# shivangchopra11/MedMoE

Measured on AMD Instinct MI355X. Metric: image-text pairs/sec at global batch 1024, higher is better.
Workload: dtype bf16; 1 GPU; cfg2: ViT-B/16 + 12-layer text tower (frozen), 8 experts top-2, 224x224x3 + 77 tokens, fwd+bwd+clip+Adam; global_batch=1024, per_gpu_batch=1024, parallelism=dp1

## Files before the change

### medmoe_amd/csrc/gemm_scores.hip

```cpp
#include "gemm_nt.h"
#include "options.h"

struct ScoresArgs {
  const bf16_t* ctx; const bf16_t* words; const int* cap_lens; const int* cap_list;
  bf16_t* a1; float* lse;
  int M, HW, HWP, Bc, T, D, n_cap;
  long long col_base, ldp, bstride;
  int skip_epi; float inv_hw;
};

template <int CTRL>
__device__ __forceinline__ float sc_dpp(float v) {
  return __builtin_bit_cast(float, __builtin_amdgcn_update_dpp(0, __builtin_bit_cast(int, v), CTRL, 0xf, 0xf, true));
}
__device__ __forceinline__ float sc_row16_sum(float v) {
  v += sc_dpp<0xB1>(v); v += sc_dpp<0x4E>(v); v += sc_dpp<0x141>(v); v += sc_dpp<0x140>(v);
  return v;
}
__device__ __forceinline__ float sc_row16_max(float v) {
  v = fmaxf(v, sc_dpp<0xB1>(v)); v = fmaxf(v, sc_dpp<0x4E>(v)); v = fmaxf(v, sc_dpp<0x141>(v)); v = fmaxf(v, sc_dpp<0x140>(v));
  return v;
}

#define SC_DPP4(OP, CTRL)                                                                                            \
  "v_" OP "_f32_dpp %0, %0, %0 " CTRL " row_mask:0xf bank_mask:0xf\n\tv_" OP "_f32_dpp %1, %1, %1 " CTRL " row_mask:0xf bank_mask:0xf\n\t" \
  "v_" OP "_f32_dpp %2, %2, %2 " CTRL " row_mask:0xf bank_mask:0xf\n\tv_" OP "_f32_dpp %3, %3, %3 " CTRL " row_mask:0xf bank_mask:0xf\n\t"
__device__ __forceinline__ void sc_row16_max4(float& a, float& b, float& c, float& d) {
  asm volatile("s_nop 1\n\t" SC_DPP4("max", "quad_perm:[1,0,3,2]") SC_DPP4("max", "quad_perm:[2,3,0,1]") SC_DPP4("max", "row_half_mirror")
               SC_DPP4("max", "row_mirror") : "+v"(a), "+v"(b), "+v"(c), "+v"(d));
}
__device__ __forceinline__ void sc_row16_sum4(float& a, float& b, float& c, float& d) {
  asm volatile("s_nop 1\n\t" SC_DPP4("add", "quad_perm:[1,0,3,2]") SC_DPP4("add", "quad_perm:[2,3,0,1]") SC_DPP4("add", "row_half_mirror")
               SC_DPP4("add", "row_mirror") : "+v"(a), "+v"(b), "+v"(c), "+v"(d));
}

template <int NTT, bool TR = false>
__global__ __launch_bounds__(512, 2) void scores512_kernel(ScoresArgs p) {
  constexpr int TP = NTT * 16;
  constexpr int WNN = (NTT == 5) ? 2 : 4;
  constexpr int WMM = 8 / WNN;
  constexpr int TMW = 16 / WMM;
  constexpr int CW = (NTT == 1) ? 4 : (NTT == 2) ? 2 : 1;
  constexpr int TNW = CW * NTT;
  constexpr int BNS = WNN * TNW * 16;
  constexpr int CAPB = WNN * CW;
  constexpr int NPIECE = (256 + BNS) / 16;
  __shared__ __attribute__((aligned(16))) char smem[NRING * SUB3];
  const int tid = threadIdx.x, lane = tid & 63, wid = tid >> 6;
  const int wm = wid % WMM, wn = wid / WMM;
  const int fr = lane & 15, g = lane >> 4;
  const int G = gridDim.x;
  const int my = xcd_remap(blockIdx.x, G);
  const int tiles_m = (p.M + 255) / 256, tiles_n = (p.n_cap + CAPB - 1) / CAPB;
  const int total = tiles_m * tiles_n;
  const int nu = p.D / 32;
  struct Tile { int m0, c0; };
  auto decode = [&](int id) -> Tile { Tile t; t.m0 = (id / tiles_n) * 256; t.c0 = (id % tiles_n) * CAPB; return t; };

  unsigned src[4];
  bool have[4];
  auto setup = [&](const Tile& t) {
#pragma unroll
    for (int i = 0; i < 4; ++i) {
      const int piece = i * 8 + wid;
      have[i] = piece < NPIECE;
      const int line = piece * 8 + (lane >> 3);
      const int lc = (lane & 7) ^ (line & 7);
      const int row = 2 * line + (lc >> 2);
      if (i < 2) src[i] = (unsigned)min(t.m0 + row, p.M - 1) * (unsigned)(p.D * 2) + (lc & 3) * 16;
      else {
        const int n = min(row - 256, BNS - 1);
        const int cj = min(t.c0 + n / TP, p.n_cap - 1), tw = min(n % TP, p.T - 1);
        src[i] = (unsigned)(p.cap_list[cj] * p.T + tw) * (unsigned)(p.D * 2) + (lc & 3) * 16;
      }
    }
  };
  auto stage = [&](int buf, int k0) {
    char* sb = smem + buf * SUB3 + wid * 1024;
#pragma unroll
    for (int i = 0; i < 4; ++i)
      if (have[i])
        __builtin_amdgcn_global_load_lds(GLB_PTR((const char*)(i < 2 ? p.ctx : p.words) + k0 * 2 + src[i]), LDS_PTR(sb + i * 8192), 16, 0, 0);
  };
  f32x4_t acc[TMW][TNW];
  auto zero_acc = [&]() __attribute__((always_inline)) {
#pragma unroll
    for (int i = 0; i < TMW; ++i)
#pragma unroll
      for (int j = 0; j < TNW; ++j) acc[i][j] = (f32x4_t){0.f, 0.f, 0.f, 0.f};
  };
  const int lane_off = (fr >> 1) * 128 + (((((fr & 1) << 2) | g) ^ ((fr >> 1) & 7)) << 4);
  const int offA_nat = (wm * TMW * 16) * 64 + lane_off;
  const int sig = ((((fr >> 2) & 1) << 1 | (fr >> 3)) << 2) | (fr & 3);
  const int pg = ((g & 1) << 1) | (g >> 1);
  const int sig_off = (sig >> 1) * 128 + (((((sig & 1) << 2) | g) ^ ((sig >> 1) & 7)) << 4);
  const int offA = TR ? (wm * TMW * 16) * 64 + sig_off : offA_nat;
  const int offB = (256 + wn * TNW * 16) * 64 + (TR ? lane_off : sig_off);
  bf16x8_t af[TMW], bf[TNW];
  auto read_frags = [&](int buf) __attribute__((always_inline)) {
    const char* sA = smem + buf * SUB3 + offA;
    const char* sB = smem + buf * SUB3 + offB;
#pragma unroll
    for (int t = 0; t < TMW; ++t) af[t] = *(const bf16x8_t*)(sA + t * 1024);
#pragma unroll
    for (int t = 0; t < TNW; ++t) bf[t] = *(const bf16x8_t*)(sB + t * 1024);
  };
  auto compute = [&]() __attribute__((always_inline)) {
#pragma unroll
    for (int tm = 0; tm < TMW; ++tm)
#pragma unroll
      for (int tn = 0; tn < TNW; ++tn)
        acc[tm][tn] = TR ? __builtin_amdgcn_mfma_f32_16x16x32_bf16(af[tm], bf[tn], acc[tm][tn], 0, 0, 0)
                         : __builtin_amdgcn_mfma_f32_16x16x32_bf16(bf[tn], af[tm], acc[tm][tn], 0, 0, 0);
  };
  auto div_hw = [&](int m, int& q, int& r) __attribute__((always_inline)) {
    q = (int)(((float)m + 0.5f) * p.inv_hw);
    r = m - q * p.HW;
    if (r < 0) { --q; r += p.HW; }
    if (r >= p.HW) { ++q; r -= p.HW; }
  };
  auto epilogue_t = [&](const Tile& t) __attribute__((always_inline)) {
#pragma unroll
    for (int c = 0; c < CW; ++c) {
      const int cj = t.c0 + wn * CW + c;
      const bool cap_ok = cj < p.n_cap && p.skip_epi != 2;
      const int cap_i = p.cap_list[min(cj, p.n_cap - 1)];
      const int cap = max(1, min(min(p.cap_lens[cap_i], p.T), TP));
      if ((NTT - 1) * 16 + fr >= cap) {
#pragma unroll
        for (int tm = 0; tm < TMW; ++tm)
#pragma unroll
          for (int r = 0; r < 4; ++r) acc[tm][c * NTT + NTT - 1][r] = -INFINITY;
      }
      if (NTT > 1 && cap <= (NTT - 1) * 16) {
#pragma unroll
        for (int tn = 0; tn < NTT - 1; ++tn)
          if (tn * 16 + fr >= cap) {
#pragma unroll
            for (int tm = 0; tm < TMW; ++tm)
#pragma unroll
              for (int r = 0; r < 4; ++r) acc[tm][c * NTT + tn][r] = -INFINITY;
          }
      }
#pragma unroll
      for (int J = 0; J < TMW / 4; ++J) {
        uint4 vv[2][NTT];
#pragma unroll
        for (int jq = 0; jq < 2; ++jq) {
          const int jp = 2 * J + jq;
          uint2 o[2][NTT];
#pragma unroll
          for (int q = 0; q < 2; ++q) {
            const int tm = 2 * jp + q;
            constexpr float L2E = 1.44269504088896f;
            float mx[4], sm[4], lse2[4];
  #pragma unroll
            for (int r = 0; r < 4; ++r) {
              mx[r] = acc[tm][c * NTT][r];
  #pragma unroll
              for (int tn = 1; tn < NTT; ++tn) mx[r] = fmaxf(mx[r], acc[tm][c * NTT + tn][r]);
            }
            sc_row16_max4(mx[0], mx[1], mx[2], mx[3]);
  #pragma unroll
            for (int r = 0; r < 4; ++r) {
              mx[r] *= L2E;
              sm[r] = 0.f;
  #pragma unroll
              for (int tn = 0; tn < NTT; ++tn) sm[r] += __builtin_amdgcn_exp2f(__builtin_fmaf(acc[tm][c * NTT + tn][r], L2E, -mx[r]));
            }
            sc_row16_sum4(sm[0], sm[1], sm[2], sm[3]);
            float lse4[4];
  #pragma unroll
            for (int r = 0; r < 4; ++r) { lse2[r] = mx[r] + __builtin_amdgcn_logf(sm[r]); lse4[r] = lse2[r] * 0.6931471805599453f; }
            typedef _Float16 h2_t __attribute__((ext_vector_type(2)));
            const h2_t lo2 = __builtin_bit_cast(h2_t, LOGP_MIN_BITS2);
  #pragma unroll
            for (int tn = 0; tn < NTT; ++tn) {
              float e[4];
  #pragma unroll
              for (int r = 0; r < 4; ++r) e[r] = __builtin_fmaf(acc[tm][c * NTT + tn][r], L2E, -lse2[r]);
              o[q][tn].x = __builtin_bit_cast(uint32_t, __builtin_elementwise_max(__builtin_bit_cast(h2_t, pack2h(e[0], e[1])), lo2));
              o[q][tn].y = __builtin_bit_cast(uint32_t, __builtin_elementwise_max(__builtin_bit_cast(h2_t, pack2h(e[2], e[3])), lo2));
            }
            const int m4 = t.m0 + wm * TMW * 16 + tm * 16 + 4 * pg;
            if (fr == 0 && m4 < p.M && cap_ok) {
              int mb, hw;
              div_hw(m4, mb, hw);
              *(float4*)(p.lse + ((long long)mb * p.Bc + cap_i) * p.HWP + hw) = make_float4(lse4[0], lse4[1], lse4[2], lse4[3]);
            }
          }
  
#pragma unroll
          for (int tn = 0; tn < NTT; ++tn) {
            auto r0 = __builtin_amdgcn_permlane32_swap(o[0][tn].x, o[1][tn].x, false, false);
            auto r1 = __builtin_amdgcn_permlane32_swap(o[0][tn].y, o[1][tn].y, false, false);
            vv[jq][tn] = make_uint4(r0[0], r1[0], r0[1], r1[1]);
          }
        }
        const int m8 = t.m0 + wm * TMW * 16 + (4 * J + (g >> 1)) * 16 + (g & 1) * 8 + 32 * (fr >> 3);
        int mb, hw;
        div_hw(min(m8, p.M - 4), mb, hw);
        const bool ok = m8 < p.M && cap_ok;
        const bool whole = hw + 8 <= p.HW;
        const bool ok2 = m8 + 4 < p.M;
        bf16_t* dst0 = p.a1 + (p.col_base + (long long)cj * TP + (fr & 7)) * p.ldp + (long long)mb * p.bstride + hw;
        bf16_t* dst2 = p.a1 + (p.col_base + (long long)cj * TP + (fr & 7)) * p.ldp + (long long)(mb + 1) * p.bstride;
#pragma unroll
        for (int tn = 0; tn < NTT; ++tn) {
#pragma unroll
          for (int i = 0; i < 2; ++i) {
            const uint4 a = vv[0][tn], b = vv[1][tn];
            uint4 y;
            if (i == 0) {
              y.x = __builtin_amdgcn_update_dpp(a.x, b.x, 0x128, 0xf, 0xC, false); y.y = __builtin_amdgcn_update_dpp(a.y, b.y, 0x128, 0xf, 0xC, false);
              y.z = __builtin_amdgcn_update_dpp(a.z, b.z, 0x128, 0xf, 0xC, false); y.w = __builtin_amdgcn_update_dpp(a.w, b.w, 0x128, 0xf, 0xC, false);
            } else {
              y.x = __builtin_amdgcn_update_dpp(b.x, a.x, 0x128, 0xf, 0x3, false); y.y = __builtin_amdgcn_update_dpp(b.y, a.y, 0x128, 0xf, 0x3, false);
              y.z = __builtin_amdgcn_update_dpp(b.z, a.z, 0x128, 0xf, 0x3, false); y.w = __builtin_amdgcn_update_dpp(b.w, a.w, 0x128, 0xf, 0x3, false);
            }
            const long long ro = (long long)(tn * 16 + 8 * i) * p.ldp;
            if (ok && whole) *(uint4*)(dst0 + ro) = y;
            else if (ok) {
              *(uint2*)(dst0 + ro) = make_uint2(y.x, y.y);
              if (ok2) *(uint2*)(dst2 + ro) = make_uint2(y.z, y.w);
            }
          }
        }
      }
    }
  };
  auto epilogue = [&](const Tile& t) __attribute__((always_inline)) -> int {
    int n_st = 0;
#pragma unroll
    for (int c = 0; c < CW; ++c) {
      const int cj = t.c0 + wn * CW + c;
      const bool cap_ok = cj < p.n_cap;
      const int cap_i = p.cap_list[min(cj, p.n_cap - 1)];
      const int cap = min(min(p.cap_lens[cap_i], p.T), TP);
#pragma unroll
      for (int tm = 0; tm < TMW; ++tm) {
        float mx = -INFINITY;
#pragma unroll
        for (int tn = 0; tn < NTT; ++tn)
#pragma unroll
          for (int r = 0; r < 4; ++r)
            if (tn * 16 + pg * 4 + r < cap) mx = fmaxf(mx, acc[tm][c * NTT + tn][r]);
        mx = fmaxf(mx, __shfl_xor(mx, 16, 64));
        mx = fmaxf(mx, __shfl_xor(mx, 32, 64));
        float sm = 0.f;
#pragma unroll
        for (int tn = 0; tn < NTT; ++tn)
#pragma unroll
          for (int r = 0; r < 4; ++r)
            sm += (tn * 16 + pg * 4 + r < cap) ? __expf(acc[tm][c * NTT + tn][r] - mx) : 0.f;
        sm += __shfl_xor(sm, 16, 64);
        sm += __shfl_xor(sm, 32, 64);
        const float lse = mx + __logf(sm);
        const int m = t.m0 + wm * TMW * 16 + tm * 16 + fr;
        const bool ok = m < p.M && cap_ok;
        const int mb = min(m, p.M - 1) / p.HW, hw = min(m, p.M - 1) - mb * p.HW;
        if (ok && g == 0) p.lse[((long long)mb * p.Bc + cap_i) * p.HWP + hw] = lse;
        bf16_t* dst = p.a1 + ((long long)mb * p.HWP + hw) * p.ldp + p.col_base + (long long)cj * TP;
        float e[NTT][4];
#pragma unroll
        for (int tn = 0; tn < NTT; ++tn)
#pragma unroll
          for (int r = 0; r < 4; ++r)
            e[tn][r] = (tn * 16 + pg * 4 + r < cap) ? fmaxf(acc[tm][c * NTT + tn][r] - lse, LOGP_MIN) : LOGP_MIN;
        uint2 o[NTT];
#pragma unroll
        for (int tn = 0; tn < NTT; ++tn) {
          o[tn].x = pack2h(e[tn][0], e[tn][1]);
          o[tn].y = pack2h(e[tn][2], e[tn][3]);
        }
#pragma unroll
        for (int j = 0; j < NTT / 2; ++j) {
          auto r0 = __builtin_amdgcn_permlane32_swap(o[2 * j].x, o[2 * j + 1].x, false, false);
          auto r1 = __builtin_amdgcn_permlane32_swap(o[2 * j].y, o[2 * j + 1].y, false, false);
          if (ok) *(uint4*)(dst + (2 * j + (g >> 1)) * 16 + (g & 1) * 8) = make_uint4(r0[0], r1[0], r0[1], r1[1]);
        }
        if ((NTT & 1) && ok) *(uint2*)(dst + (NTT - 1) * 16 + pg * 4) = o[NTT - 1];
        n_st += NTT;
      }
    }
    return n_st + TMW * CW;
  };

  if (my >= total) return;
  const int my_tiles = (total - my + G - 1) / G;
  Tile ct = decode(my);
  setup(ct);
  int lid = my, lk = 0, wb = 0, rb = 0;
  bool lmore = true;
  int drain = 0;
  auto issue = [&]() __attribute__((always_inline)) {
    if (lmore) {
      stage(wb, lk * 32);
      wb = (wb + 1) & 3;
      if (++lk == nu) {
        lk = 0; lid += G;
        if (lid < total) { const Tile lt = decode(lid); setup(lt); } else lmore = false;
      }
    }
  };
  const int my_pieces = (have[0] ? 1 : 0) + (have[1] ? 1 : 0) + (have[2] ? 1 : 0) + (have[3] ? 1 : 0);
  auto wait_third_newest = [&]() __attribute__((always_inline)) {
    if (drain > 0 || !lmore) { asm volatile("s_waitcnt vmcnt(0)" ::: "memory"); if (drain > 0) --drain; }
    else if (my_pieces == 4) asm volatile("s_waitcnt vmcnt(8)" ::: "memory");
    else if (my_pieces == 3) asm volatile("s_waitcnt vmcnt(6)" ::: "memory");
    else asm volatile("s_waitcnt vmcnt(4)" ::: "memory");
  };
  const int grp = __builtin_amdgcn_readfirstlane(wid >> 2);
  zero_acc();
  issue(); issue(); issue();
  asm volatile("s_waitcnt vmcnt(0)" ::: "memory");
  __builtin_amdgcn_s_barrier();
  asm volatile("" ::: "memory");
  auto seg_barrier = [&]() {
    __builtin_amdgcn_sched_barrier(0);
    __builtin_amdgcn_s_barrier();
    __builtin_amdgcn_sched_barrier(0);
    asm volatile("" ::: "memory");
  };
  auto load_seg = [&]() __attribute__((always_inline)) {
    read_frags(rb);
    rb = (rb + 1) & 3;
    issue();
    if (grp == 1) wait_third_newest();
    seg_barrier();
  };
  auto body = [&](bool last) __attribute__((always_inline)) {
    compute();
    if (grp == 0) { wait_third_newest(); seg_barrier(); }
    if (last) {
      if (p.skip_epi != 1) { if constexpr (TR) epilogue_t(ct); else epilogue(ct); }
      zero_acc();
      drain = 3;
    }
    if (grp == 1) seg_barrier();
    load_seg();
  };
  if (grp == 1) seg_barrier();
  load_seg();
  for (int ti = 0; ti < my_tiles; ++ti) {
    for (int k = 1; k < nu; ++k) body(false);
    body(true);
    if (ti + 1 < my_tiles) ct = decode(my + (ti + 1) * G);
  }
  if (grp == 0) seg_barrier();
}

int g_use_scores512 = 1, g_scores_skip_epi = 0;

static ScoresArgs sc_args(const void* ctx, const void* words, const int* cap_lens, const int* cap_list, void* out, float* lse, long long M,
                          int HW, int Bc, int T, int D, int n_cap, long long col_base, long long ldp, long long bstride) {
  ScoresArgs p;
  p.ctx = (const bf16_t*)ctx; p.words = (const bf16_t*)words; p.cap_lens = cap_lens; p.cap_list = cap_list;
  p.a1 = (bf16_t*)out; p.lse = lse;
  p.M = (int)M; p.HW = HW; p.HWP = ((HW + 15) / 16) * 16; p.Bc = Bc; p.T = T; p.D = D; p.n_cap = n_cap;
  p.col_base = col_base; p.ldp = ldp; p.bstride = bstride; p.skip_epi = g_scores_skip_epi; p.inv_hw = 1.0f / (float)HW;
  return p;
}

template <bool TR>
static void sc_launch(const ScoresArgs& p, int ntt, hipStream_t stream) {
  const int tiles_m = (p.M + 255) / 256;
#define SC(N_, CAPB_) { const int grid = min(tiles_m * ((p.n_cap + CAPB_ - 1) / CAPB_), 256); \
                        hipLaunchKernelGGL((scores512_kernel<N_, TR>), dim3(grid), dim3(512), 0, stream, p); }
  switch (ntt) { case 1: SC(1, 16) break; case 2: SC(2, 8) break; case 3: SC(3, 4) break; case 4: SC(4, 4) break; default: SC(5, 2) break; }
#undef SC
}

extern "C" int medmoe_local_scores_t(const void* ctx, const void* words, const int* cap_lens, void* lpT, float* lse, int B, int Bc,
                                     int HW, int T, int D, const int* cap_list, int n_cap, int ntt, long long row_base, long long ld,
                                     long long bstride, hipStream_t stream) {
  if (!ctx || !words || !cap_lens || !lpT || !lse || !cap_list) return MM_ERR_ARG;
  if (B <= 0 || Bc <= 0 || HW < 4 || (HW % 4) || T <= 0 || n_cap <= 0 || n_cap > Bc || ntt < 1 || ntt > 5 || row_base < 0) return MM_ERR_SHAPE;
  const long long M = (long long)B * HW;
  const int HWP = ((HW + 15) / 16) * 16;
  if ((D % 32) || D < 128 || M * D * 2 >= (1ll << 32) || (long long)Bc * T * D * 2 >= (1ll << 32) || (ld % 4) || (bstride % 4) || ld < HWP || bstride < HWP) return MM_ERR_SHAPE;
  sc_launch<true>(sc_args(ctx, words, cap_lens, cap_list, lpT, lse, M, HW, Bc, T, D, n_cap, row_base, ld, bstride), ntt, stream);
  return mm_check_launch();
}

bool mm_launch_scores512(const void* ctx, const void* words, const int* cap_lens, void* a1, float* lse, int B, int Bc, int HW, int T,
                         int D, const int* cap_list, int n_cap, int ntt, long long col_base, long long ldp, hipStream_t stream) {
  const long long M = (long long)B * HW;
  if (!g_use_scores512 || (D % 32) || D < 128 || M < 1024 || M * D * 2 >= (1ll << 32) || (long long)Bc * T * D * 2 >= (1ll << 32)) return false;
  sc_launch<false>(sc_args(ctx, words, cap_lens, cap_list, a1, lse, M, HW, Bc, T, D, n_cap, col_base, ldp, 0), ntt, stream);
  return true;
}
```

### medmoe_amd/csrc/options.h

```cpp
#pragma once
#include "common.h"

MM_HIDDEN extern int g_use_nt256;
MM_HIDDEN extern int g_use_nt512;
MM_HIDDEN extern int g_use_tn512;
MM_HIDDEN extern int g_tn_rows;
MM_HIDDEN extern int g_nt_max_grid;
MM_HIDDEN extern int g_use_scores512;
MM_HIDDEN extern int g_use_nt4w;
MM_HIDDEN extern int g_use_tn4w;
MM_HIDDEN extern int g_tn_min_rows;
MM_HIDDEN extern int g_tn_rows4w;
MM_HIDDEN extern int g_attn_resident;
MM_HIDDEN extern int g_scores_skip_epi;
MM_HIDDEN extern int g_sa_rows;
MM_HIDDEN extern int g_attn_rt13;
MM_HIDDEN extern int g_ln_one_row;
MM_HIDDEN extern int g_use_nt_direct;
```

### medmoe_amd/csrc/options.hip

```cpp
#include "options.h"

extern "C" int medmoe_set_option(int key, int value) {
  if (key == 1) { g_use_nt256 = value; return MM_OK; }
  if (key == 2) { g_use_nt512 = value; return MM_OK; }
  if (key == 3) { g_use_tn512 = value; return MM_OK; }
  if (key == 4 && value >= 256) { g_tn_rows = value; return MM_OK; }
  if (key == 5 && value >= 1 && value <= 256) { g_nt_max_grid = value; return MM_OK; }
  if (key == 6) { g_use_scores512 = value; return MM_OK; }
  if (key == 7) { g_use_nt4w = value; return MM_OK; }
  if (key == 8) { g_use_tn4w = value; return MM_OK; }
  if (key == 9 && value >= 64) { g_tn_min_rows = value; return MM_OK; }
  if (key == 10 && value >= 0) { g_tn_rows4w = value; return MM_OK; }
  if (key == 11) { g_attn_resident = value; return MM_OK; }
  if (key == 12) { g_scores_skip_epi = value; return MM_OK; }
  if (key == 13 && value >= 0) { g_sa_rows = value; return MM_OK; }
  if (key == 15 && (value == 0 || value == 448 || value == 512)) { g_attn_rt13 = value; return MM_OK; }
  if (key == 16) { g_ln_one_row = value; return MM_OK; }
  if (key == 17) { g_use_nt_direct = value; return MM_OK; }
  return MM_ERR_ARG;
}

MM_HIDDEN long long g_mm_nondet = 0;
extern "C" long long medmoe_nondet_launches() { return g_mm_nondet; }
```

Baseline: 4758 pairs/s.

## Group score tiles by row blocks and add LDS-staged full-line transposed output writes

Changes the tile decode of the transposed local-scores kernel so consecutive tile ids sweep a group of row tiles (default 4) before moving to the next caption column block, aiming for better L2 reuse of the context rows. Adds an optional LINES path that stages each wave's transposed output in LDS and writes whole aligned 128-byte lines to global memory, replacing scattered 8-byte stores. The LINES path is off by default (option 14), while row grouping is on by default for the transposed entry point. The staging path adds LDS usage and complex alignment logic.

After: 4784 pairs/s (median of 6 runs). No clear change (+0.5%).

```diff
diff --git a/medmoe_amd/csrc/gemm_scores.hip b/medmoe_amd/csrc/gemm_scores.hip
--- a/medmoe_amd/csrc/gemm_scores.hip
+++ b/medmoe_amd/csrc/gemm_scores.hip
@@ -7,6 +7,7 @@
   int M, HW, HWP, Bc, T, D, n_cap;
   long long col_base, ldp, bstride;
   int skip_epi; float inv_hw;
+  int rgroup;
 };
 
 template <int CTRL>
@@ -34,7 +35,7 @@
                SC_DPP4("add", "row_mirror") : "+v"(a), "+v"(b), "+v"(c), "+v"(d));
 }
 
-template <int NTT, bool TR = false>
+template <int NTT, bool TR = false, bool LINES = false>
 __global__ __launch_bounds__(512, 2) void scores512_kernel(ScoresArgs p) {
   constexpr int TP = NTT * 16;
   constexpr int WNN = (NTT == 5) ? 2 : 4;
@@ -46,6 +47,8 @@
   constexpr int CAPB = WNN * CW;
   constexpr int NPIECE = (256 + BNS) / 16;
   __shared__ __attribute__((aligned(16))) char smem[NRING * SUB3];
+  static_assert(!LINES || (TR && TMW == 8), "LINES: the transposed output of a 128-region wave tile");
+  __shared__ __attribute__((aligned(16))) char sc_stage[LINES ? 8 * 4096 : 16];
   const int tid = threadIdx.x, lane = tid & 63, wid = tid >> 6;
   const int wm = wid % WMM, wn = wid / WMM;
   const int fr = lane & 15, g = lane >> 4;
@@ -55,7 +58,12 @@
   const int total = tiles_m * tiles_n;
   const int nu = p.D / 32;
   struct Tile { int m0, c0; };
-  auto decode = [&](int id) -> Tile { Tile t; t.m0 = (id / tiles_n) * 256; t.c0 = (id % tiles_n) * CAPB; return t; };
+  const int rgroup = max(1, min(p.rgroup, tiles_m));
+  auto decode = [&](int id) -> Tile {
+    const int per = rgroup * tiles_n, s = id / per, rem = id - s * per;
+    const int rows = min(rgroup, tiles_m - s * rgroup), c = rem / rows;
+    Tile t; t.m0 = (s * rgroup + rem - c * rows) * 256; t.c0 = c * CAPB; return t;
+  };
 
   unsigned src[4];
   bool have[4];
@@ -120,6 +128,35 @@
     if (r >= p.HW) { ++q; r -= p.HW; }
   };
   auto epilogue_t = [&](const Tile& t) __attribute__((always_inline)) {
+    [[maybe_unused]] int lenA = 0, lenB = 0;
+    [[maybe_unused]] long long gA = 0, gB = 0;
+    [[maybe_unused]] unsigned voA = 0, voB = 0;
+    [[maybe_unused]] int posA = 0, posB = 0;
+    [[maybe_unused]] unsigned ldsW = 0, ldsA = 0, ldsB0 = 0, ldsB1 = 0;
+    if constexpr (LINES) {
+      const int m0w = t.m0 + wm * TMW * 16;
+      int mbw, hw0;
+      div_hw(min(m0w, p.M - 4), mbw, hw0);
+      mbw = __builtin_amdgcn_readfirstlane(mbw); hw0 = __builtin_amdgcn_readfirstlane(hw0);
+      const int LA = m0w < p.M ? min(128, p.HW - hw0) : 0;
+      const int LB = (LA < 128 && m0w + LA < p.M) ? 128 - LA : 0;
+      lenA = 2 * LA; lenB = 2 * LB;
+      const long long row0 = (p.col_base + (long long)(t.c0 + wn * CW) * TP) * p.ldp;
+      gA = 2 * (row0 + (long long)mbw * p.bstride + hw0) - 128;
+      gB = 2 * (row0 + (long long)(mbw + 1) * p.bstride) - 128;
+      const unsigned a0 = (unsigned)(unsigned long long)p.a1;
+      const int r8 = lane >> 3, j16 = (lane & 7) * 16;
+      const unsigned rowb = 2u * (unsigned)r8 * (unsigned)p.ldp;
+      const int alA = (int)((a0 + (unsigned)gA + rowb) & 127u), alB = (int)((a0 + (unsigned)gB + rowb) & 127u);
+      posA = j16 - alA; posB = j16 - alB;
+      voA = rowb + 128u + (unsigned)posA; voB = rowb + 128u + (unsigned)posB;
+      const unsigned st = (unsigned)(wid * 4096);
+      ldsA = st + r8 * 256 + ((j16 + 16 * r8) & 255);
+      ldsB0 = st + r8 * 256 + ((lenA + posB + alA + 16 * r8) & 255);
+      ldsB1 = st + r8 * 256 + ((lenA + posB + 8 + alA + 16 * r8) & 255);
+      const int alW = (int)((a0 + (unsigned)gA + 2u * (unsigned)fr * (unsigned)p.ldp) & 127u);
+      ldsW = alW + 16 * fr + (g >> 1) * 32 + (g & 1) * 16;
+    }
 #pragma unroll
     for (int c = 0; c < CW; ++c) {
       const int cj = t.c0 + wn * CW + c;
@@ -142,9 +179,10 @@
               for (int r = 0; r < 4; ++r) acc[tm][c * NTT + tn][r] = -INFINITY;
           }
       }
+      uint4 vq[TMW / 4][2][NTT];
 #pragma unroll
       for (int J = 0; J < TMW / 4; ++J) {
-        uint4 vv[2][NTT];
+        uint4 (&vv)[2][NTT] = vq[J];
 #pragma unroll
         for (int jq = 0; jq < 2; ++jq) {
           const int jp = 2 * J + jq;
@@ -197,6 +235,7 @@
             vv[jq][tn] = make_uint4(r0[0], r1[0], r0[1], r1[1]);
           }
         }
+        if constexpr (LINES) continue;
         const int m8 = t.m0 + wm * TMW * 16 + (4 * J + (g >> 1)) * 16 + (g & 1) * 8 + 32 * (fr >> 3);
         int mb, hw;
         div_hw(min(m8, p.M - 4), mb, hw);
@@ -223,6 +262,50 @@
             else if (ok) {
               *(uint2*)(dst0 + ro) = make_uint2(y.x, y.y);
               if (ok2) *(uint2*)(dst2 + ro) = make_uint2(y.z, y.w);
+            }
+          }
+        }
+      }
+      if constexpr (LINES) {
+        if (cap_ok && lenA > 0) {
+          char* const stg = sc_stage;
+          char* const outc = (char*)p.a1 + 2 * (long long)c * TP * p.ldp;
+          const bool two = lenB > 0;
+          auto put = [&](char* q, uint4 y, int pos, int len) __attribute__((always_inline)) {
+            const bool lo = pos >= 0 && pos + 8 <= len, hi = pos + 8 >= 0 && pos + 16 <= len;
+            if (lo && hi) *(uint4*)q = y;
+            else if (lo) *(uint2*)q = make_uint2(y.x, y.y);
+            else if (hi) *(uint2*)(q + 8) = make_uint2(y.z, y.w);
+          };
+#pragma unroll
+          for (int tn = 0; tn < NTT; ++tn) {
+#pragma unroll
+            for (int J = 0; J < 2; ++J)
+#pragma unroll
+              for (int jq = 0; jq < 2; ++jq) {
+                const uint4 v = vq[J][jq][tn];
+                char* const rw = stg + wid * 4096 + fr * 256;
+                *(uint2*)(rw + ((ldsW + J * 128 + jq * 64) & 255)) = make_uint2(v.x, v.y);
+                *(uint2*)(rw + ((ldsW + J * 128 + jq * 64 + 8) & 255)) = make_uint2(v.z, v.w);
+              }
+#pragma unroll
+            for (int h = 0; h < 2; ++h) {
+              const long long ro = 2 * (long long)(tn * 16 + h * 8) * p.ldp;
+#pragma unroll
+              for (int k = 0; k < 3; ++k) {
+                if (k * 128 - 120 >= lenA) break;
+                const uint4 y = *(const uint4*)(stg + (ldsA ^ (((h + k) & 1) << 7)) + h * 2048);
+                put(outc + gA + ro + k * 128 + voA, y, posA + k * 128, lenA);
+              }
+              if (two) {
+#pragma unroll
+                for (int k = 0; k < 3; ++k) {
+                  if (k * 128 - 120 >= lenB) break;
+                  const uint2 y0 = *(const uint2*)(stg + (ldsB0 ^ (((h + k) & 1) << 7)) + h * 2048);
+                  const uint2 y1 = *(const uint2*)(stg + (ldsB1 ^ (((h + k) & 1) << 7)) + h * 2048);
+                  put(outc + gB + ro + k * 128 + voB, make_uint4(y0.x, y0.y, y1.x, y1.y), posB + k * 128, lenB);
+                }
+              }
             }
           }
         }
@@ -350,7 +433,7 @@
   if (grp == 0) seg_barrier();
 }
 
-int g_use_scores512 = 1, g_scores_skip_epi = 0;
+int g_use_scores512 = 1, g_scores_skip_epi = 0, g_scores_lines = 0, g_scores_rgroup = 4;
 
 static ScoresArgs sc_args(const void* ctx, const void* words, const int* cap_lens, const int* cap_list, void* out, float* lse, long long M,
                           int HW, int Bc, int T, int D, int n_cap, long long col_base, long long ldp, long long bstride) {
@@ -359,15 +442,19 @@
   p.a1 = (bf16_t*)out; p.lse = lse;
   p.M = (int)M; p.HW = HW; p.HWP = ((HW + 15) / 16) * 16; p.Bc = Bc; p.T = T; p.D = D; p.n_cap = n_cap;
   p.col_base = col_base; p.ldp = ldp; p.bstride = bstride; p.skip_epi = g_scores_skip_epi; p.inv_hw = 1.0f / (float)HW;
+  p.rgroup = 1;
   return p;
 }
 
 template <bool TR>
 static void sc_launch(const ScoresArgs& p, int ntt, hipStream_t stream) {
   const int tiles_m = (p.M + 255) / 256;
-#define SC(N_, CAPB_) { const int grid = min(tiles_m * ((p.n_cap + CAPB_ - 1) / CAPB_), 256); \
-                        hipLaunchKernelGGL((scores512_kernel<N_, TR>), dim3(grid), dim3(512), 0, stream, p); }
-  switch (ntt) { case 1: SC(1, 16) break; case 2: SC(2, 8) break; case 3: SC(3, 4) break; case 4: SC(4, 4) break; default: SC(5, 2) break; }
+  const bool lines = TR && g_scores_lines && p.HW >= 124 && (p.ldp % 8) == 0 && ntt <= 4;
+#define SC(N_, CAPB_, L_) { const int grid = min(tiles_m * ((p.n_cap + CAPB_ - 1) / CAPB_), 256); \
+                            hipLaunchKernelGGL((scores512_kernel<N_, TR, L_>), dim3(grid), dim3(512), 0, stream, p); }
+#define SCL(N_, CAPB_) { if constexpr (TR) { if (lines) SC(N_, CAPB_, true) else SC(N_, CAPB_, false) } else SC(N_, CAPB_, false) }
+  switch (ntt) { case 1: SCL(1, 16) break; case 2: SCL(2, 8) break; case 3: SCL(3, 4) break; case 4: SCL(4, 4) break; default: SC(5, 2, false) break; }
+#undef SCL
 #undef SC
 }
 
@@ -379,7 +466,9 @@
   const long long M = (long long)B * HW;
   const int HWP = ((HW + 15) / 16) * 16;
   if ((D % 32) || D < 128 || M * D * 2 >= (1ll << 32) || (long long)Bc * T * D * 2 >= (1ll << 32) || (ld % 4) || (bstride % 4) || ld < HWP || bstride < HWP) return MM_ERR_SHAPE;
-  sc_launch<true>(sc_args(ctx, words, cap_lens, cap_list, lpT, lse, M, HW, Bc, T, D, n_cap, row_base, ld, bstride), ntt, stream);
+  ScoresArgs p = sc_args(ctx, words, cap_lens, cap_list, lpT, lse, M, HW, Bc, T, D, n_cap, row_base, ld, bstride);
+  p.rgroup = g_scores_rgroup;
+  sc_launch<true>(p, ntt, stream);
   return mm_check_launch();
 }
 
diff --git a/medmoe_amd/csrc/options.h b/medmoe_amd/csrc/options.h
--- a/medmoe_amd/csrc/options.h
+++ b/medmoe_amd/csrc/options.h
@@ -14,6 +14,8 @@
 MM_HIDDEN extern int g_attn_resident;
 MM_HIDDEN extern int g_scores_skip_epi;
 MM_HIDDEN extern int g_sa_rows;
+MM_HIDDEN extern int g_scores_lines;
+MM_HIDDEN extern int g_scores_rgroup;
 MM_HIDDEN extern int g_attn_rt13;
 MM_HIDDEN extern int g_ln_one_row;
 MM_HIDDEN extern int g_use_nt_direct;
diff --git a/medmoe_amd/csrc/options.hip b/medmoe_amd/csrc/options.hip
--- a/medmoe_amd/csrc/options.hip
+++ b/medmoe_amd/csrc/options.hip
@@ -14,9 +14,11 @@
   if (key == 11) { g_attn_resident = value; return MM_OK; }
   if (key == 12) { g_scores_skip_epi = value; return MM_OK; }
   if (key == 13 && value >= 0) { g_sa_rows = value; return MM_OK; }
+  if (key == 14) { g_scores_lines = value; return MM_OK; }
   if (key == 15 && (value == 0 || value == 448 || value == 512)) { g_attn_rt13 = value; return MM_OK; }
   if (key == 16) { g_ln_one_row = value; return MM_OK; }
   if (key == 17) { g_use_nt_direct = value; return MM_OK; }
+  if (key == 18 && value >= 1) { g_scores_rgroup = value; return MM_OK; }
   return MM_ERR_ARG;
 }
 
```
